# RoyiAvital/QuadraticProgramSolver

Hardware: AMD Instinct MI355X
Metric: ADMM iterations/sec (higher is better)
Workload: dtype f64

## Files before the change

quadraticprogramsolver_amd/csrc/k_loop.hip:

```cpp
#include <cstdlib>

#include "qps_kernels.h"
#include "wave_reduce.h"
#include <hip/hip_ext.h>

namespace qps {

namespace {

template <typename T> __device__ __forceinline__ T wave_sum(T v) { return wave_sum_all(v); }
__device__ __forceinline__ unsigned long long absbits(double v) { return (unsigned long long)__double_as_longlong(fabs(v)); }
__device__ __forceinline__ unsigned long long wave_max_u64(unsigned long long v) {
#pragma unroll
    for (int o = 32; o > 0; o >>= 1) { unsigned long long t = __shfl_xor(v, o, 64); v = t > v ? t : v; }
    return v;
}

template <typename T, int RB, int TRI, int THREADS>
__global__ __launch_bounds__(THREADS) void k_gemv_rows(const T* __restrict__ S, int64_t ld, const T* __restrict__ v,
                                                   T* __restrict__ out, const T* __restrict__ out0, T alpha, T beta,
                                                   int r0, int c0, int c1, BatchStride bs) {
    using V = typename VecOf<T>::type;
    if (bs.active && !bs.active[blockIdx.y]) return;
    S += (int64_t)blockIdx.y * bs.mat; v += (int64_t)blockIdx.y * bs.vin; out += (int64_t)blockIdx.y * bs.vout;
    if (out0) out0 += (int64_t)blockIdx.y * bs.vout;
    constexpr int VN = VecOf<T>::N;
// ... 9 lines not shown
    const T* Srow = S + (int64_t)rb * ld;
#pragma unroll 4
    for (int c = cb + tid * VN; c < ce; c += CHUNK) {
        const V vv = *reinterpret_cast<const V*>(v + c);
        const T* vp = reinterpret_cast<const T*>(&vv);
#pragma unroll
        for (int i = 0; i < RB; ++i) {
            typedef T NV __attribute__((ext_vector_type(VN)));
            const NV* src = reinterpret_cast<const NV*>(Srow + (int64_t)i * ld + c);
            const NV a = (TRI == 0) ? __builtin_nontemporal_load(src) : *src;
            T ap[VN];
#pragma unroll
            for (int e = 0; e < VN; ++e) ap[e] = a[e];
#pragma unroll
            for (int e = 0; e < VN; ++e) {
                bool ok = true;
                if (TRI == 1) ok = (c + e) <= (rb + i);
                if (TRI == 2) ok = (c + e) >= (rb + i);
                acc[i] += ok ? ap[e] * vp[e] : T(0);
            }
        }
    }
    __shared__ T red[THREADS / 64][RB];
#pragma unroll
    for (int i = 0; i < RB; ++i) acc[i] = wave_sum(acc[i]);
    if ((tid & 63) == 0) {
#pragma unroll
        for (int i = 0; i < RB; ++i) red[tid >> 6][i] = acc[i];
    }
    __syncthreads();
// ... 27 lines not shown
        T w = ca * va[rbase + i];
        if (vb) w += cb * vb[rbase + i];
        typedef T NV __attribute__((ext_vector_type(VN)));
        const NV a = __builtin_nontemporal_load(reinterpret_cast<const NV*>(Sp + (int64_t)i * ld));
#pragma unroll
        for (int e = 0; e < VN; ++e) acc[e] += a[e] * w;
    }
    V o;
    T* op = reinterpret_cast<T*>(&o);
#pragma unroll
    for (int e = 0; e < VN; ++e) op[e] = acc[e];
    *reinterpret_cast<V*>(part + (int64_t)rt * part_ld + c) = o;
}

template <typename T>
__global__ __launch_bounds__(256) void k_colsum(const T* __restrict__ part, int64_t part_ld, int ntiles,
                                                const T* __restrict__ a0, T s0, const T* __restrict__ a1, T s1,
                                                T* __restrict__ out, int ncols, BatchStride bs) {
    using V = typename VecOf<T>::type;
    constexpr int VN = VecOf<T>::N;
    if (bs.active && !bs.active[blockIdx.y]) return;
    part += (int64_t)blockIdx.y * bs.mat; out += (int64_t)blockIdx.y * bs.vout;
    if (a0) a0 += (int64_t)blockIdx.y * bs.vin;
    if (a1) a1 += (int64_t)blockIdx.y * bs.vin;
    constexpr int COLS = 128 / (int)sizeof(T);
    constexpr int CL = COLS / VN;
    constexpr int TL = 256 / CL;
    const int cl = threadIdx.x % CL, tl = threadIdx.x / CL;
    const int c = blockIdx.x * COLS + cl * VN;
    T acc[VN];
#pragma unroll
    for (int e = 0; e < VN; ++e) acc[e] = T(0);
    if (c < ncols) {
        int t = tl;
        for (; t + 7 * TL < ntiles; t += 8 * TL) {
            V v[8];
#pragma unroll
            for (int j = 0; j < 8; ++j) v[j] = *reinterpret_cast<const V*>(part + (int64_t)(t + TL * j) * part_ld + c);
#pragma unroll
// ... 10 lines not shown
            for (int e = 0; e < VN; ++e) acc[e] += vp[e];
        }
    }
    __shared__ T red[TL][COLS + 1];
#pragma unroll
    for (int e = 0; e < VN; ++e) red[tl][cl * VN + e] = acc[e];
    __syncthreads();
    constexpr int PL = 256 / COLS;
    static_assert(TL % PL == 0 && (PL == 16 || PL == 8), "slab lanes per output");
    const int o = threadIdx.x / PL, pl = threadIdx.x % PL;
    T s = T(0);
#pragma unroll
    for (int k = 0; k < TL / PL; ++k) s += red[pl * (TL / PL) + k][o];
    s = (PL == 16) ? row16_sum_last(s) : oct_sum_all(s);
    const int oc = blockIdx.x * COLS + o;
    if (pl == PL - 1 && oc < ncols) {
        T r = s;
        if (a0) r += s0 * a0[oc];
        if (a1) r += s1 * a1[oc];
        out[oc] = r;
    }
}

template <typename T>
__global__ __launch_bounds__(256) void k_admm_update(int NP, int MP, const T* __restrict__ xx, const T* __restrict__ zz,
                                                     T* __restrict__ x, T* __restrict__ xp, T* __restrict__ z,
                                                     T* __restrict__ zp, T* __restrict__ y, const T* __restrict__ l,
                                                     const T* __restrict__ u, T alpha, T rho) {
    const int i = blockIdx.x * 256 + threadIdx.x;
    const T alpha1 = T(1) - alpha, rho1 = T(1) / rho;
    if (i < NP) {
        const T xo = x[i];
        xp[i] = xo;
        x[i] = alpha * xx[i] + alpha1 * xo;
    }
    if (i < MP) {
// ... 34 lines not shown
            v[4] = max(v[4], absbits((double)Px[i]));
            v[5] = max(v[5], absbits((double)Aty[i]));
            v[6] = max(v[6], absbits((double)q[i]));
            if (!dual_only) v[7] = max(v[7], absbits((double)(x[i] - xp[i])));
        }
    }
#pragma unroll
    for (int k = 0; k < 9; ++k) {
        v[k] = wave_max_u64(v[k]);
        if ((threadIdx.x & 63) == 0 && v[k] != 0ull) atomicMax(&slots[k], v[k]);
    }
}

__device__ __forceinline__ double jmax(double a, double b) { return (isnan(a) || isnan(b)) ? (double)NAN : (a > b ? a : b); }

__global__ void k_check_decide(const unsigned long long* __restrict__ slots, double* __restrict__ res, CheckScalars cs,
                               const double* __restrict__ rho_arr, const double* __restrict__ rhorho_arr,
                               const int* __restrict__ active) {
    if (threadIdx.x != 0) return;
    const int b = blockIdx.x;
    if (active && !active[b]) return;
    slots += (int64_t)b * 16; res += (int64_t)b * 8;
    if (rho_arr) { cs.rho = rho_arr[b]; cs.rhorho = rhorho_arr[b]; cs.convFlag = 1; }
    double nv[9];
    for (int k = 0; k < 9; ++k) nv[k] = __longlong_as_double((long long)slots[k]);
    const double MIN_VAL_RHO = 1e-3, MAX_VAL_RHO = 1e6;
    const double normResPrim = nv[0], normResDual = nv[1];
    const double maxNormPrim = jmax(nv[2], nv[3]);
    const double maxNormDual = jmax(jmax(nv[4], nv[5]), nv[6]);
    double rhorho = cs.rhorho;
    if (cs.adptRho) {
        const double numeratorVal = normResPrim * maxNormDual;
        const double denominatorVal = normResDual * maxNormPrim;
        const double t = cs.rho * sqrt(numeratorVal / denominatorVal);
        rhorho = t > MAX_VAL_RHO ? MAX_VAL_RHO : (t < MIN_VAL_RHO ? MIN_VAL_RHO : t);
    }
    const double epsPrim = cs.epsAbs + cs.epsRel * maxNormPrim;
    const double epsDual = cs.epsAbs + cs.epsRel * maxNormDual;
    int flag = cs.convFlag;
    if ((normResPrim < epsPrim) && (normResDual < epsDual)) flag = 3;
    if ((nv[7] <= cs.epsAdmm) && (nv[8] <= cs.epsAdmm)) flag = 2;
    res[0] = normResPrim; res[1] = normResDual; res[2] = maxNormPrim; res[3] = maxNormDual;
    res[4] = rhorho; res[5] = (double)flag; res[6] = nv[7]; res[7] = nv[8];
}

template <typename T> __global__ void k_fill(T* p, int64_t n, T v) {
    int64_t i = (int64_t)blockIdx.x * 256 + threadIdx.x;
    if (i < n) p[i] = v;
}
template <typename T> __global__ void k_convert(const double* __restrict__ s, T* __restrict__ d, int64_t n) {
    int64_t i = (int64_t)blockIdx.x * 256 + threadIdx.x;
    if (i < n) d[i] = (T)s[i];
}
template <typename T> __global__ void k_convert_back(const T* __restrict__ s, double* __restrict__ d, int64_t n) {
    int64_t i = (int64_t)blockIdx.x * 256 + threadIdx.x;
    if (i < n) d[i] = (double)s[i];
}

// ... 59 lines not shown
}

template <typename T>
void check_convergence(hipStream_t st, int n, int m, const T* Ax, const T* Px, const T* Aty, const T* q, const T* x,
                       const T* xp, const T* z, const T* zp, unsigned long long* scratch, double* res_dev, CheckScalars cs,
                       int dual_only, BatchStride bs, const double* rho_arr, const double* rhorho_arr) {
    if (!dual_only) (void)hipMemsetAsync(scratch, 0, 16 * sizeof(unsigned long long) * bs.count, st);
    const int N = n > m ? n : m;
    int blocks = (N + 255) / 256;
    if (blocks > 1024) blocks = 1024;
    if (blocks < 1) blocks = 1;
    hipLaunchKernelGGL((k_check_norms<T>), dim3(blocks, bs.count), dim3(256), 0, st, n, m, Ax, Px, Aty, q, x, xp, z, zp, scratch, dual_only, bs);
    hipLaunchKernelGGL(k_check_decide, dim3(bs.count), dim3(64), 0, st, scratch, res_dev, cs, rho_arr, rhorho_arr, bs.active);
}

template <typename T> void fill(hipStream_t st, T* p, int64_t n, T v) {
    if (n <= 0) return;
    hipLaunchKernelGGL((k_fill<T>), dim3((unsigned)((n + 255) / 256)), dim3(256), 0, st, p, n, v);
}
template <typename T> void convert_copy(hipStream_t st, const double* src, T* dst, int64_t n) {
    if (n <= 0) return;
    hipLaunchKernelGGL((k_convert<T>), dim3((unsigned)((n + 255) / 256)), dim3(256), 0, st, src, dst, n);
}
template <typename T> void convert_back(hipStream_t st, const T* src, double* dst, int64_t n) {
    if (n <= 0) return;
    hipLaunchKernelGGL((k_convert_back<T>), dim3((unsigned)((n + 255) / 256)), dim3(256), 0, st, src, dst, n);
}

#define INST(T)                                                                                                              \
    template void gemv_rows<T>(hipStream_t, const T*, int64_t, const T*, T*, const T*, T, T, int, int, int, int, int, BatchStride); \
    template int gemv_cols_partial<T>(hipStream_t, const T*, int64_t, const T*, const T*, T, T, T*, int64_t, int, int);      \
    template void colsum<T>(hipStream_t, const T*, int64_t, int, const T*, T, const T*, T, T*, int, BatchStride);            \
    template void admm_update<T>(hipStream_t, int, int, const T*, const T*, T*, T*, T*, T*, T*, const T*, const T*, T, T);   \
    template void check_convergence<T>(hipStream_t, int, int, const T*, const T*, const T*, const T*, const T*, const T*,    \
                                       const T*, const T*, unsigned long long*, double*, CheckScalars, int, BatchStride,     \
                                       const double*, const double*);                                                        \
    template void fill<T>(hipStream_t, T*, int64_t, T);                                                                      \
    template void convert_copy<T>(hipStream_t, const double*, T*, int64_t);                                                  \
    template void convert_back<T>(hipStream_t, const T*, double*, int64_t);
INST(double)
INST(float)
#undef INST

}
```

quadraticprogramsolver_amd/csrc/qps_capi.hip:

```cpp
#include "ldl_symbolic.h"
#include <atomic>
#include <limits>
#include <memory>
#include <thread>

#include "batch_schedule.h"
#include "dense_chol.h"
#include "qps_internal.h"
#include "spmv_layout.h"
#include "qps_kernels.h"
#include "qps_ldl.h"
#include "qps_polish.h"
#include "qps_proxqp.h"

using namespace qps;

namespace qps {
namespace {
constexpr size_t kPinnedBytes = 512, kRecycleBlockMax = (size_t)512 << 20;
constexpr int kRecyclePerDevice = 4;
std::mutex g_res_mu;
std::vector<HandleResources> g_res[kMaxDevices];
std::atomic<int> g_cus[kMaxDevices];
}
// ... 95 lines not shown
template <typename T> struct DenseSolver : SolverBase {
    int NP = 0, MP = 0;
    T *A = nullptr, *P = nullptr, *q = nullptr, *l = nullptr, *u = nullptr;
    T *PI = nullptr, *AA = nullptr, *M = nullptr, *S = nullptr, *tmp = nullptr, *dinv = nullptr; int* fail = nullptr;
    T *x = nullptr, *xp = nullptr, *z = nullptr, *zp = nullptr, *y = nullptr, *xx = nullptr, *zz = nullptr, *tt = nullptr, *yv = nullptr;
    T *part = nullptr, *part2 = nullptr, *sw_part = nullptr, *Ax = nullptr, *Px = nullptr, *Aty = nullptr;
    T* At = nullptr; void* small_out = nullptr; void* small_out_host = nullptr; bool small_ok = false;
    StreamLease lease; Arena arena;
    double* stage_mat = nullptr; int64_t stage_mat_count = 0;
    int pass_slabs = 0, pass_rpw = 0;
    unsigned long long* scratch = nullptr; double* res_dev = nullptr; double* res_host = nullptr; double* stage = nullptr;
    bool have_AA = false, factor_valid = false; double fac_rho = 0, fac_sigma = 0; int fac_nb = 0;
    int nb = 2048; int part_tiles = 0; int num_factorizations = 0;
    unsigned long long* pub = nullptr; unsigned* abort_dev = nullptr; unsigned sweep_epoch = 0; bool blocked_off = false, fac_premul = false;
    bool use_blocked() const { return !blocked_off && trsv_blocked_supported<T>(NP, nb); }
    struct IterGraph { int count; const void* xa; double rho, sigma, alpha; int nb; hipGraphExec_t exec; };
    std::vector<IterGraph> graphs;
    bool graphs_disabled = false;
    void drop_graphs() { for (auto& gr : graphs) (void)hipGraphExecDestroy(gr.exec); graphs.clear(); }
    hipGraphExec_t iter_graph(int count, T* xa, T* xb, double rho, double sigma, double alpha) {
        for (auto& gr : graphs) if (gr.count == count && gr.xa == xa && gr.rho == rho && gr.sigma == sigma && gr.alpha == alpha && gr.nb == nb) return gr.exec;
        if (graphs_disabled) return nullptr;
        if (graphs.size() >= 8) drop_graphs();
        hipGraph_t graph = nullptr; hipGraphExec_t exec = nullptr;
        if (hipStreamBeginCapture(st, hipStreamCaptureModeThreadLocal) != hipSuccess) { (void)hipGetLastError(); graphs_disabled = true; return nullptr; }
        for (int k = 0; k < count; ++k) {
            colsum<T>(st, part, NP, pass_slabs, xa, (T)sigma, q, T(-1), tt, NP);
            sweeps();
            apass<T>(st, false, A, NP, NP, MP, xx, xa, xb, z, y, l, u, (T)alpha, (T)rho, part, part2, NP, scratch);
            std::swap(xa, xb);
// ... 32 lines not shown
            Ax = ar.take<T>(MP); Px = ar.take<T>(NP); Aty = ar.take<T>(NP);
            scratch = ar.take<unsigned long long>(16); res_dev = ar.take<double>(16);
            pub = ar.take<unsigned long long>(trsv_blocked_pub_words<T>(NP));
            abort_dev = reinterpret_cast<unsigned*>(res_dev + 14);
            stage = ar.take<double>((int64_t)NP + 2 * (int64_t)MP + 64);
            if (small_ok) { At = ar.take<T>((int64_t)NP * MP); small_out = ar.take<double>(32); }
            if (stage_mat_count > 0) stage_mat = ar.take<double>(stage_mat_count);
        };
        layout(arena);
        st = prof.st = lease.acquire(device, arena.planned());
        HandleResources& res = lease.res;
        char* const recycled = res.block; res.block = nullptr;
        arena.commit(st, recycled, res.block_bytes);
        layout(arena);
        res_host = reinterpret_cast<double*>(res.pinned);
        small_out_host = small_ok ? reinterpret_cast<char*>(res.pinned) + 16 * sizeof(double) : nullptr;
        const double s = sizeof(T);
        cat_atw = prof.category("gemv_cols(A'w)", s * ((double)m * n + m + n));
        cat_colsum = prof.category("colsum(rhs)", s * ((double)part_tiles * n + 3.0 * n));
        cat_fwd = prof.category("trsv_forward", s * ((double)n * (n + 1) / 2 + 2.0 * n));
        cat_bwd = prof.category("trsv_backward", s * ((double)n * (n + 1) / 2 + 2.0 * n));
        cat_ax = prof.category("gemv_rows(Ax~)", s * ((double)m * n + m + n));
        cat_upd = prof.category("admm_update", s * (3.0 * n + 7.0 * m));
        cat_chk = prof.category("check_convergence", s * (2.0 * m * n + (double)n * n + 4.0 * n + 4.0 * m));
        cat_pass = prof.category("apass(fused A-pass)", s * ((double)m * n + 3.0 * n + 6.0 * m));
        cat_passchk = prof.category("apass(check variant)", s * ((double)m * n + 4.0 * n + 6.0 * m));
        cat_sweep = prof.category("sweeps(fused fwd+bwd, triangle read once)", s * ((double)n * (n + 1) / 2 + 2.0 * n + (double)sweep_fused_slabs<T>(NP) * n));
        cat_xsum = prof.category("colsum(x~ slabs)", s * ((double)sweep_fused_slabs<T>(NP) * n + n));
        cat_small = prof.category("admm_small(whole loop in one launch; bytes per iteration)", s * ((double)m * n + (double)n * n) + s * (6.0 * n + 10.0 * m));
    }
// ... 132 lines not shown
            ii = it;
            const double t2s = now_s();
            PolishReport prs;
            if (p.polish) polish_dense<T>(st, n, m, NP, MP, P, A, q, l, u, y, x, part, p, &prs);
            download_vec(x, xh, n);
            if (info) {
                info->convFlag = convFlag; info->iterations = ii; info->numRefactor = nref; info->cgIterations = 0;
                info->rhoFinal = rho; info->rhoProposed = rhorho; info->resPrim = resP; info->resDual = resD;
                info->tSetup = t1 - t0; info->tLoop = t2s - t1; info->tRefactor = tref;
                info->polishFlag = prs.flag; info->polishIterations = prs.minresIterations; info->tPolish = prs.seconds;
                info->trsvBlock = nb; info->sweepVariant = 4;
            }
            return false;
        }
        const bool fused = pass_slabs > 0 && p.loopVariant != 1;
        int rhs_slabs = 0;
        static const int graph_env = [] { const char* e = getenv("QPS_GRAPH"); return e ? atoi(e) : -1; }();
        const bool use_graph = fused && prof.level == 0 && p.numItrConv >= 3 && !fac_premul && (graph_env >= 0 ? graph_env != 0 : NP <= 2048);
        for (ii = 1; ii <= p.numIterations; ++ii) {
            bool changed = false;
            if (p.adptRho && ((rhorho * p.fctrRho < rho) || (rhorho > p.fctrRho * rho))) {
                rho = rhorho; ++nref; changed = true;
                const double ta = now_s();
                factorize(rho, sigma, false);
                tref += now_s() - ta;
            }
            const bool check = (ii % p.numItrConv == 0);
            if (use_graph && !changed && !check && rhs_slabs == pass_slabs) {
                int run = std::min(p.numItrConv - ii % p.numItrConv, p.numIterations - ii + 1) & ~1;
                hipGraphExec_t ge = run >= 2 ? iter_graph(run, x, xp, rho, sigma, alpha) : nullptr;
// ... 5 lines not shown
            }
            if (!fused) {
                linear_solve(rho, sigma);
                {
                    ProfScope ps(prof, cat_upd, 2);
                    admm_update<T>(st, NP, MP, xx, zz, x, xp, z, zp, y, l, u, (T)alpha, (T)rho);
                }
                if (check) {
                    ProfScope ps(prof, cat_chk, 2);
                    gemv_rows<T>(st, A, NP, x, Ax, nullptr, T(1), T(0), 0, MP, 0, NP, 0);
                    gemv_rows<T>(st, P, NP, x, Px, nullptr, T(1), T(0), 0, NP, 0, NP, 0);
                    gemv_cols_partial<T>(st, A, NP, y, nullptr, T(1), T(0), part, NP, MP, NP);
                    colsum<T>(st, part, NP, part_tiles, nullptr, T(0), nullptr, T(0), Aty, NP);
                    CheckScalars cs{p.epsAbs, p.epsRel, epsAdmm, rho, rhorho, p.adptRho, convFlag};
                    check_convergence<T>(st, (int)n, (int)m, Ax, Px, Aty, q, x, xp, z, zp, scratch, res_dev, cs);
                }
            } else {
                if (changed && rhs_slabs > 0) {
                    ProfScope ps(prof, cat_atw, 2);
                    rhs_slabs = gemv_cols_partial<T>(st, A, NP, z, y, (T)rho, T(-1), part, NP, MP, NP);
                }
                prof_iter = ii;
                {
                    ProfLaunchScope ps(prof, cat_colsum, sample_lvl(29));
                    colsum<T>(st, part, NP, rhs_slabs, x, (T)sigma, q, T(-1), tt, NP);
                }
                sweeps();
                if (check) HIPC(hipMemsetAsync(scratch, 0, 16 * sizeof(unsigned long long), st));
                {
                    const int lvl = (prof.level == 1 && (check || ii % 50 != 38)) ? 3 : 1;
                    ProfLaunchScope ps(prof, check ? cat_passchk : cat_pass, lvl);
                    apass<T>(st, check, A, NP, NP, MP, xx, x, xp, z, y, l, u, (T)alpha, (T)rho, part, part2, NP, scratch);
                }
                std::swap(x, xp);
                rhs_slabs = pass_slabs;
                if (check) {
                    ProfScope ps(prof, cat_chk, 2);
                    colsum<T>(st, part2, NP, pass_slabs, nullptr, T(0), nullptr, T(0), Aty, NP);
                    gemv_rows<T>(st, P, NP, x, Px, nullptr, T(1), T(0), 0, NP, 0, NP, 0);
                    CheckScalars cs{p.epsAbs, p.epsRel, epsAdmm, rho, rhorho, p.adptRho, convFlag};
                    check_convergence<T>(st, (int)n, (int)m, Ax, Px, Aty, q, x, xp, z, zp, scratch, res_dev, cs, 1);
                }
            }
            if (check) {
                HIPC(hipMemcpyAsync(res_host, res_dev, 15 * sizeof(double), hipMemcpyDeviceToHost, st));
                HIPC(hipStreamSynchronize(st));
                prof.harvest();
                if (sweep_gave_up(true)) return true;
                resP = res_host[0]; resD = res_host[1]; rhorho = res_host[4]; convFlag = (int)res_host[5];
                if (convFlag != QPS_CONV_NUM_ITR) break;
            }
        }
        HIPC(hipStreamSynchronize(st));
        prof.harvest();
        if (sweep_gave_up()) return true;
        const double t2 = now_s();
        PolishReport pr;
        if (p.polish) polish_dense<T>(st, n, m, NP, MP, P, A, q, l, u, y, x, part, p, &pr);
        download_vec(x, xh, n);
        if (info) {
            info->convFlag = convFlag; info->iterations = ii > p.numIterations ? p.numIterations : ii;
// ... 104 lines not shown
    const double denominatorVal = res[8 * bd + 1] * res[8 * bp + 2];
    const double t = rho * std::sqrt(numeratorVal / denominatorVal);
    return t > MAX_VAL_RHO ? MAX_VAL_RHO : (t < MIN_VAL_RHO ? MIN_VAL_RHO : t);
}

template <typename T> struct BatchedDenseSolver : BatchSolverBase {
    StreamLease lease; DeviceOwner mem; hipStream_t st = nullptr;
    int NP = 0, MP = 0, nb = 0, slabs = 0, rpw = 0, part_tiles = 0;
    T *A = nullptr, *P = nullptr, *q = nullptr, *l = nullptr, *u = nullptr, *PI = nullptr, *AA = nullptr, *M = nullptr, *S = nullptr,
      *tmp = nullptr, *dinv = nullptr;
    T *x = nullptr, *xp = nullptr, *xres = nullptr, *z = nullptr, *y = nullptr, *xx = nullptr, *tt = nullptr, *yv = nullptr, *part = nullptr,
      *part2 = nullptr, *part_tmp = nullptr, *sw_part = nullptr, *Px = nullptr, *Aty = nullptr;
    int* fail = nullptr; int* d_active = nullptr; double *d_rho = nullptr, *d_rhorho = nullptr;
    unsigned long long* scratch = nullptr; double* res_dev = nullptr; double* res_host = nullptr; double* stage = nullptr;
    int* h_int = nullptr; double* h_dbl = nullptr;
    bool have_AA = false; double fac_sigma = -1; int fac_nb = -1; std::vector<double> fac_rho;
    char* sb_args = nullptr; void* sb_host = nullptr;
    int cat_pass = 0, cat_sweep = 0;

    BatchedDenseSolver(int dev, int cnt, int64_t n_, int64_t m_) {
        device = dev; n = n_; m = m_; count = cnt;
        HIPC(hipSetDevice(device));
        st = prof.st = lease.acquire(device);
        NP = roundup(n, 64); MP = roundup(m, 64);
        slabs = apass_plan<T>(NP, MP, &rpw, count);
        {
            const double s = sizeof(T), c = cnt;
            cat_pass = prof.category("apass(fused A-pass, batched)", c * s * ((double)m * n + 3.0 * n + 6.0 * m));
            cat_sweep = prof.category("sweeps(fused fwd+bwd, batched, triangle read once)", c * s * ((double)n * (n + 1) / 2 + 2.0 * n));
        }
        part_tiles = gemv_cols_tiles(MP);
        const int64_t nn = (int64_t)NP * NP, c = count;
        A = mem.dalloc<T>(c * MP * NP, st); P = mem.dalloc<T>(c * nn, st); PI = mem.dalloc<T>(c * nn, st); AA = mem.dalloc<T>(c * nn, st); M = mem.dalloc<T>(c * nn, st);
        S = mem.dalloc<T>(c * nn, st); tmp = mem.dalloc<T>(c * nn, st); dinv = mem.dalloc<T>(c * (int64_t)(NP / 64) * 4096, st);
        q = mem.dalloc<T>(c * NP, st); l = mem.dalloc<T>(c * MP, st); u = mem.dalloc<T>(c * MP, st);
        x = mem.dalloc<T>(c * NP, st); xp = mem.dalloc<T>(c * NP, st); xres = mem.dalloc<T>(c * NP, st); xx = mem.dalloc<T>(c * NP, st); tt = mem.dalloc<T>(c * NP, st);
        yv = mem.dalloc<T>(c * NP, st); Px = mem.dalloc<T>(c * NP, st); Aty = mem.dalloc<T>(c * NP, st); z = mem.dalloc<T>(c * MP, st); y = mem.dalloc<T>(c * MP, st);
        int rpw1 = 0;
        const int64_t part_slabs = std::max<int64_t>(std::max<int64_t>(c * slabs, apass_plan<T>(NP, MP, &rpw1, 1)), std::max(part_tiles, 1));
        part = mem.dalloc<T>(part_slabs * NP, st); part2 = mem.dalloc<T>(c * slabs * NP, st); part_tmp = mem.dalloc<T>((int64_t)std::max(part_tiles, 1) * NP, st);
        const int sw_slabs = sweep_fused_slabs<T>(NP, count); sw_part = mem.dalloc<T>(c * std::max(sw_slabs, 1) * NP, st);
        fail = mem.dalloc<int>(count + 4, st); d_active = mem.dalloc<int>(count + 4, st); d_rho = mem.dalloc<double>(count + 4, st); d_rhorho = mem.dalloc<double>(count + 4, st);
        scratch = mem.dalloc<unsigned long long>(16 * c, st); res_dev = mem.dalloc<double>(8 * c, st);
        res_host = mem.pinned<double>(8 * c); h_int = mem.pinned<int>(count + 4); h_dbl = mem.pinned<double>(2 * (count + 4));
        stage = mem.dalloc<double>(std::max<int64_t>((int64_t)MP * NP, nn) + 64, st);
    }
    ~BatchedDenseSolver() override {
        (void)hipSetDevice(device);
        (void)hipStreamSynchronize(st);
        prof.release_events();
    }
    std::unique_ptr<FastUploader> loader;
    void put_vec(const double* h, T* d, int64_t cnt_) {
        if (cnt_ <= 0) return;
        if (!loader) loader.reset(new FastUploader(st, device));
        loader->copy(stage, h, sizeof(double) * (size_t)cnt_);
        convert_copy<T>(st, stage, d, cnt_);
    }
    void put_matrix(const double* h, int rows, int cols, T* d) {
// ... 46 lines not shown
        else for (int b : todo) { ch.at(b).form(sigma, p.rho, rebuild, rebuild); ch.at(b).factor(nb); }
        ch.check(what, "", h_int, count, &todo);
        have_AA = true; fac_sigma = sigma; fac_nb = nb;
        for (int b : todo) fac_rho[b] = p.rho;
        for (int b = 0; b < count; ++b) put_vec(xh + (int64_t)b * n, x + (int64_t)b * NP, n);
        loader.reset();
        HIPC(hipMemsetAsync(z, 0, sizeof(T) * (size_t)count * MP, st));
        HIPC(hipMemsetAsync(y, 0, sizeof(T) * (size_t)count * MP, st));
        push_state(rho, rhorho, active);
        const double t1 = now_s();
        BatchStride bsS; bsS.count = count; bsS.mat = (int64_t)NP * NP; bsS.vin = NP; bsS.vout = NP; bsS.active = d_active;
        BatchStride bsC; bsC.count = count; bsC.mat = (int64_t)slabs * NP; bsC.vin = NP; bsC.vout = NP; bsC.active = d_active;
        BatchStride bsK; bsK.count = count; bsK.vin = NP; bsK.vout = MP; bsK.active = d_active;
        PassBatch pb; pb.count = count; pb.slabs = slabs; pb.rho_arr = d_rho; pb.active = d_active;
        int rhs_slabs = 0, nactive = count, ii = 0;
        const int nblk = (NP + nb - 1) / nb;
        if (p.loopVariant == 0 && nblk == 1 && admm_small_batch_supported<T>(NP, MP)) {
            const size_t ab = admm_small_args_bytes(), ob = admm_small_out_bytes();
            if (!sb_host) { sb_args = mem.dalloc<char>((int64_t)(ab + ob) * count + 64, st); sb_host = mem.pinned<char>((ab + ob) * (size_t)count + 64); }
            char* args_h = static_cast<char*>(sb_host); char* outs_h = args_h + ab * count;
            char* args_d = sb_args; char* outs_d = sb_args + ab * count;
            std::vector<int> it(count, 0);
            HIPC(hipMemsetAsync(xp, 0, sizeof(T) * (size_t)count * NP, st));
            while (nactive > 0) {
                for (int b = 0; b < count; ++b)
                    admm_small_args_set(args_h, b, (int)n, (int)m, NP, MP, it[b], active[b] ? p.numIterations : it[b], p.numItrConv, p.adptRho, rho[b], rhorho[b],
                                        sigma, alpha, p.epsAbs, p.epsRel, epsAdmm, p.fctrRho);
                HIPC(hipMemcpyAsync(args_d, args_h, ab * count, hipMemcpyHostToDevice, st));
                admm_small_batch<T>(st, count, NP, MP, args_d, A, P, S, q, l, u, x, xp, z, y, outs_d);
                HIPC(hipMemcpyAsync(outs_h, outs_d, ob * count, hipMemcpyDeviceToHost, st));
// ... 42 lines not shown
                    if (rhs_slabs > 0) {
                        T* pb_ = part + (int64_t)b * slabs * NP;
                        gemv_cols_partial<T>(st, A + (int64_t)b * MP * NP, NP, z + (int64_t)b * MP, y + (int64_t)b * MP, (T)rho[b], T(-1), part_tmp, NP, MP, NP);
                        colsum<T>(st, part_tmp, NP, part_tiles, nullptr, T(0), nullptr, T(0), pb_, NP);
                        if (slabs > 1) HIPC(hipMemsetAsync(pb_ + NP, 0, sizeof(T) * (size_t)(slabs - 1) * NP, st));
                    }
                }
                ch.check(what, "", h_int, count, together ? &all : &changed);
                push_state(rho, rhorho, active);
                const double dt = (now_s() - ta) / changed.size();
                for (int b : changed) tref[b] += dt;
            }
            const bool check = (ii % p.numItrConv == 0);
            colsum<T>(st, part, NP, rhs_slabs, x, (T)sigma, q, T(-1), tt, NP, bsC);
            ch.sweeps(nb, tt, yv, xx, sw_part, bsS, {&prof, cat_sweep, (prof.level == 1 && ii % 50 == 13) ? 1 : 2});
            if (check) HIPC(hipMemsetAsync(scratch, 0, 16 * sizeof(unsigned long long) * count, st));
            {
                ProfLaunchScope ps(prof, cat_pass, (prof.level == 1 && !check && ii % 50 == 38) ? 1 : (check ? 3 : 2));
                apass<T>(st, check, A, NP, NP, MP, xx, x, xp, z, y, l, u, (T)alpha, T(1), part, part2, NP, scratch, pb);
            }
            std::swap(x, xp);
            rhs_slabs = slabs;
            if (check) {
                colsum<T>(st, part2, NP, slabs, nullptr, T(0), nullptr, T(0), Aty, NP, bsC);
                BatchStride bsP = bsS; bsP.mat = (int64_t)NP * NP;
                gemv_rows<T>(st, P, NP, x, Px, nullptr, T(1), T(0), 0, NP, 0, NP, 0, bsP);
                CheckScalars cs{p.epsAbs, p.epsRel, epsAdmm, 0.0, 0.0, p.adptRho, QPS_CONV_NUM_ITR};
                check_convergence<T>(st, (int)n, (int)m, (const T*)nullptr, Px, Aty, q, x, xp, z, z, scratch, res_dev, cs, 1, bsK, d_rho, d_rhorho);
                HIPC(hipMemcpyAsync(res_host, res_dev, 8 * sizeof(double) * count, hipMemcpyDeviceToHost, st));
                HIPC(hipStreamSynchronize(st));
                prof.harvest();
                bool any_done = false;
                for (int b = 0; b < count; ++b) {
                    if (!active[b]) continue;
                    const double* r = res_host + 8 * b;
                    resP[b] = r[0]; resD[b] = r[1]; rhorho[b] = r[4]; conv[b] = (int)r[5];
                    if (conv[b] != QPS_CONV_NUM_ITR) {
                        active[b] = 0; iters[b] = ii; --nactive; any_done = true;
                        HIPC(hipMemcpyAsync(xres + (int64_t)b * NP, x + (int64_t)b * NP, sizeof(T) * NP, hipMemcpyDeviceToDevice, st));
                    }
                }
                push_state(rho, rhorho, active);
                (void)any_done;
            }
        }
// ... 1266 lines not shown
```

quadraticprogramsolver_amd/csrc/qps_internal.h:

```cpp
#pragma once
#include <hip/hip_runtime.h>

#include <algorithm>
#include <chrono>
#include <cmath>
#include <cstdio>
#include <cstring>
#include <mutex>
#include <string>
#include <system_error>
#include <thread>
#include <vector>

#include "../../include/qps.h"

namespace qps {

struct QpsError { int code; std::string msg; QpsError(int c, std::string m) : code(c), msg(std::move(m)) {} };

inline double now_s() { return std::chrono::duration<double>(std::chrono::steady_clock::now().time_since_epoch()).count(); }
inline int roundup(int64_t v, int q) { return (int)(((v + q - 1) / q) * q); }

struct KernelStat { double seconds = 0; int64_t launches = 0; double algo_bytes = 0; };

// ... 27 lines not shown
        for (auto& p : pending) { (void)hipEventDestroy(p.a); (void)hipEventDestroy(p.b); }
        pool.clear(); pending.clear();
    }
    ~Profiler() { for (auto e : pool) (void)hipEventDestroy(e); for (auto& p : pending) { (void)hipEventDestroy(p.a); (void)hipEventDestroy(p.b); } }
};
struct ProfLaunchScope {
    Profiler& p; int cat; hipEvent_t a, b; bool active;
    ProfLaunchScope(Profiler& pr, int c, int lvl);
    ~ProfLaunchScope();
};
struct ProfScope {
    Profiler& p; int cat; hipEvent_t a; bool active;
    ProfScope(Profiler& pr, int c, int lvl) : p(pr), cat(c), a(nullptr), active(pr.on(lvl)) { if (active) p.begin(cat, a); }
    ~ProfScope() { if (active) p.end(cat, a); }
};

#define HIPC(expr)                                                                                            \
    do {                                                                                                      \
        hipError_t e_ = (expr);                                                                               \
        if (e_ != hipSuccess) {                                                                               \
            char b_[512]; snprintf(b_, sizeof b_, "%s failed: %s (%s:%d)", #expr, hipGetErrorString(e_), __FILE__, __LINE__); \
            throw QpsError(e_ == hipErrorOutOfMemory ? QPS_ERR_OUT_OF_MEMORY : QPS_ERR_HIP, b_);               \
        }                                                                                                     \
    } while (0)

struct DeviceOwner {
    std::vector<void*> dev, host;
    DeviceOwner() = default;
    DeviceOwner(const DeviceOwner&) = delete;
    DeviceOwner& operator=(const DeviceOwner&) = delete;
// ... 151 lines not shown
```

quadraticprogramsolver_amd/csrc/qps_kernels.h:

```cpp
#pragma once
#ifndef QPS_NT_SLABS
#define QPS_NT_SLABS 1
#endif
#include <hip/hip_runtime.h>
#include <stdint.h>

#include <atomic>
#include <thread>

namespace qps {

constexpr int kMaxDevices = 64;
int current_device();
int device_cu_count(int device);
struct PerDeviceOnce {
    std::atomic<unsigned char> state[kMaxDevices] = {};
    template <typename F> void once(int dev, F&& f) {
        if (dev < 0 || dev >= kMaxDevices) { f(); return; }
        if (state[dev].load(std::memory_order_acquire) == 2) return;
        unsigned char expect = 0;
        if (state[dev].compare_exchange_strong(expect, 1, std::memory_order_acq_rel)) { f(); state[dev].store(2, std::memory_order_release); return; }
        while (state[dev].load(std::memory_order_acquire) != 2) std::this_thread::yield();
    }
};
// ... 19 lines not shown

template <typename T>
void colsum(hipStream_t st, const T* part, int64_t part_ld, int ntiles, const T* a0, T s0, const T* a1, T s1,
            T* out, int ncols, BatchStride bs = BatchStride());

template <typename T>
void admm_update(hipStream_t st, int NP, int MP, const T* xx, const T* zz, T* x, T* xp, T* z, T* zp, T* y,
                 const T* l, const T* u, T alpha, T rho);

struct CheckScalars { double epsAbs, epsRel, epsAdmm, rho, rhorho; int adptRho; int convFlag; };
template <typename T>
void check_convergence(hipStream_t st, int n, int m, const T* Ax, const T* Px, const T* Aty, const T* q, const T* x,
                       const T* xp, const T* z, const T* zp, unsigned long long* scratch , double* res_dev,
                       CheckScalars cs, int dual_only = 0, BatchStride bs = BatchStride(), const double* rho_arr = nullptr,
                       const double* rhorho_arr = nullptr);

template <typename T> int apass_plan(int NP, int MP, int* rows_per_wg, int count = 1);
template <typename T> int apass_max_np();
struct PassBatch { int count = 1; int slabs = 0; const double* rho_arr = nullptr; const int* active = nullptr; int pq_me = 0; };
template <typename T>
void apass(hipStream_t st, bool check, const T* A, int64_t ld, int NP, int MP, const T* xx, const T* x_old, T* x_new, T* z,
           T* y, const T* l, const T* u, T alpha, T rho, T* part, T* part2, int64_t part_ld, unsigned long long* slots,
           PassBatch pb = PassBatch());
template <typename T> int apass_proxqp_slabs(int NP, int MP);
template <typename T>
int apass_kkt(hipStream_t st, const T* A, int64_t ld, int NP, int MP, const T* vx, const T* vlam, const T* mask, T delta, T* out_lam,
              T* part, int64_t part_ld);
template <typename T>
int apass_proxqp(hipStream_t st, const T* G, int64_t ld, int NP, int MP, int me, const T* x, T* x_scratch, T* slack, T* dual,
                 const T* g, T rho, T* part, int64_t part_ld);
// ... 106 lines not shown
```

Measured before the change: 14510.

## Fuse convergence-check colsum, P*x gemv and decide into one epilogue kernel

Adds a k_check_epilogue kernel that, in one launch, reduces the A'y partial sums, computes P*x with double-buffered loads, folds in the dual-residual max norms, and has the last workgroup (chosen by an atomic ticket) run the convergence decision. It writes results straight into mapped pinned host memory and resets the slot scratch itself, so the memset and the device-to-host copy can be skipped on later checks. It also switches the untriangular gemv inner loop to explicit FMA. This removes several kernel launches and a memcpy per check iteration, at the cost of a more complex kernel that relies on cross-workgroup atomic ordering and on zero-copy host writes.

```diff
diff --git a/quadraticprogramsolver_amd/csrc/k_loop.hip b/quadraticprogramsolver_amd/csrc/k_loop.hip
--- a/quadraticprogramsolver_amd/csrc/k_loop.hip
+++ b/quadraticprogramsolver_amd/csrc/k_loop.hip
@@ -10,6 +10,8 @@
 
 template <typename T> __device__ __forceinline__ T wave_sum(T v) { return wave_sum_all(v); }
 __device__ __forceinline__ unsigned long long absbits(double v) { return (unsigned long long)__double_as_longlong(fabs(v)); }
+__device__ __forceinline__ double fmadd(double a, double b, double c) { return __builtin_fma(a, b, c); }
+__device__ __forceinline__ float fmadd(float a, float b, float c) { return __builtin_fmaf(a, b, c); }
 __device__ __forceinline__ unsigned long long wave_max_u64(unsigned long long v) {
 #pragma unroll
     for (int o = 32; o > 0; o >>= 1) { unsigned long long t = __shfl_xor(v, o, 64); v = t > v ? t : v; }
@@ -49,6 +51,7 @@
             for (int e = 0; e < VN; ++e) ap[e] = a[e];
 #pragma unroll
             for (int e = 0; e < VN; ++e) {
+                if (TRI == 0) { acc[i] = fmadd(ap[e], vp[e], acc[i]); continue; }
                 bool ok = true;
                 if (TRI == 1) ok = (c + e) <= (rb + i);
                 if (TRI == 2) ok = (c + e) >= (rb + i);
@@ -106,15 +109,10 @@
 }
 
 template <typename T>
-__global__ __launch_bounds__(256) void k_colsum(const T* __restrict__ part, int64_t part_ld, int ntiles,
-                                                const T* __restrict__ a0, T s0, const T* __restrict__ a1, T s1,
-                                                T* __restrict__ out, int ncols, BatchStride bs) {
+__device__ __forceinline__ T colsum_body(const T* __restrict__ part, int64_t part_ld, int ntiles, const T* __restrict__ a0, T s0,
+                                         const T* __restrict__ a1, T s1, T* __restrict__ out, int ncols, int* owner_col) {
     using V = typename VecOf<T>::type;
     constexpr int VN = VecOf<T>::N;
-    if (bs.active && !bs.active[blockIdx.y]) return;
-    part += (int64_t)blockIdx.y * bs.mat; out += (int64_t)blockIdx.y * bs.vout;
-    if (a0) a0 += (int64_t)blockIdx.y * bs.vin;
-    if (a1) a1 += (int64_t)blockIdx.y * bs.vin;
     constexpr int COLS = 128 / (int)sizeof(T);
     constexpr int CL = COLS / VN;
     constexpr int TL = 256 / CL;
@@ -155,12 +153,26 @@
     for (int k = 0; k < TL / PL; ++k) s += red[pl * (TL / PL) + k][o];
     s = (PL == 16) ? row16_sum_last(s) : oct_sum_all(s);
     const int oc = blockIdx.x * COLS + o;
+    *owner_col = -1;
+    T r = s;
     if (pl == PL - 1 && oc < ncols) {
-        T r = s;
         if (a0) r += s0 * a0[oc];
         if (a1) r += s1 * a1[oc];
         out[oc] = r;
-    }
+        *owner_col = o;
+    }
+    return r;
+}
+template <typename T>
+__global__ __launch_bounds__(256) void k_colsum(const T* __restrict__ part, int64_t part_ld, int ntiles,
+                                                const T* __restrict__ a0, T s0, const T* __restrict__ a1, T s1,
+                                                T* __restrict__ out, int ncols, BatchStride bs) {
+    if (bs.active && !bs.active[blockIdx.y]) return;
+    part += (int64_t)blockIdx.y * bs.mat; out += (int64_t)blockIdx.y * bs.vout;
+    if (a0) a0 += (int64_t)blockIdx.y * bs.vin;
+    if (a1) a1 += (int64_t)blockIdx.y * bs.vin;
+    int owner;
+    (void)colsum_body<T>(part, part_ld, ntiles, a0, s0, a1, s1, out, ncols, &owner);
 }
 
 template <typename T>
@@ -225,6 +237,26 @@
 
 __device__ __forceinline__ double jmax(double a, double b) { return (isnan(a) || isnan(b)) ? (double)NAN : (a > b ? a : b); }
 
+__device__ __forceinline__ void check_decide_body(const double* nv, const CheckScalars& cs, double* __restrict__ res) {
+    const double MIN_VAL_RHO = 1e-3, MAX_VAL_RHO = 1e6;
+    const double normResPrim = nv[0], normResDual = nv[1];
+    const double maxNormPrim = jmax(nv[2], nv[3]);
+    const double maxNormDual = jmax(jmax(nv[4], nv[5]), nv[6]);
+    double rhorho = cs.rhorho;
+    if (cs.adptRho) {
+        const double numeratorVal = normResPrim * maxNormDual;
+        const double denominatorVal = normResDual * maxNormPrim;
+        const double t = cs.rho * sqrt(numeratorVal / denominatorVal);
+        rhorho = t > MAX_VAL_RHO ? MAX_VAL_RHO : (t < MIN_VAL_RHO ? MIN_VAL_RHO : t);
+    }
+    const double epsPrim = cs.epsAbs + cs.epsRel * maxNormPrim;
+    const double epsDual = cs.epsAbs + cs.epsRel * maxNormDual;
+    int flag = cs.convFlag;
+    if ((normResPrim < epsPrim) && (normResDual < epsDual)) flag = 3;
+    if ((nv[7] <= cs.epsAdmm) && (nv[8] <= cs.epsAdmm)) flag = 2;
+    res[0] = normResPrim; res[1] = normResDual; res[2] = maxNormPrim; res[3] = maxNormDual;
+    res[4] = rhorho; res[5] = (double)flag; res[6] = nv[7]; res[7] = nv[8];
+}
 __global__ void k_check_decide(const unsigned long long* __restrict__ slots, double* __restrict__ res, CheckScalars cs,
                                const double* __restrict__ rho_arr, const double* __restrict__ rhorho_arr,
                                const int* __restrict__ active) {
@@ -235,24 +267,120 @@
     if (rho_arr) { cs.rho = rho_arr[b]; cs.rhorho = rhorho_arr[b]; cs.convFlag = 1; }
     double nv[9];
     for (int k = 0; k < 9; ++k) nv[k] = __longlong_as_double((long long)slots[k]);
-    const double MIN_VAL_RHO = 1e-3, MAX_VAL_RHO = 1e6;
-    const double normResPrim = nv[0], normResDual = nv[1];
-    const double maxNormPrim = jmax(nv[2], nv[3]);
-    const double maxNormDual = jmax(jmax(nv[4], nv[5]), nv[6]);
-    double rhorho = cs.rhorho;
-    if (cs.adptRho) {
-        const double numeratorVal = normResPrim * maxNormDual;
-        const double denominatorVal = normResDual * maxNormPrim;
-        const double t = cs.rho * sqrt(numeratorVal / denominatorVal);
-        rhorho = t > MAX_VAL_RHO ? MAX_VAL_RHO : (t < MIN_VAL_RHO ? MIN_VAL_RHO : t);
-    }
-    const double epsPrim = cs.epsAbs + cs.epsRel * maxNormPrim;
-    const double epsDual = cs.epsAbs + cs.epsRel * maxNormDual;
-    int flag = cs.convFlag;
-    if ((normResPrim < epsPrim) && (normResDual < epsDual)) flag = 3;
-    if ((nv[7] <= cs.epsAdmm) && (nv[8] <= cs.epsAdmm)) flag = 2;
-    res[0] = normResPrim; res[1] = normResDual; res[2] = maxNormPrim; res[3] = maxNormDual;
-    res[4] = rhorho; res[5] = (double)flag; res[6] = nv[7]; res[7] = nv[8];
+    check_decide_body(nv, cs, res);
+}
+
+constexpr int CE_RB = 4;
+constexpr int CE_UC = 4;
+template <typename T, bool WIDE>
+__global__ __launch_bounds__(256) void k_check_epilogue(const T* __restrict__ part2, int64_t part_ld, int ntiles, T* __restrict__ Aty,
+                                                        const T* __restrict__ P, int64_t ld, const T* __restrict__ x, T* __restrict__ Px,
+                                                        const T* __restrict__ q, int n, int NP, unsigned long long* __restrict__ slots,
+                                                        double* __restrict__ res, const unsigned* __restrict__ abort_src,
+                                                        unsigned* __restrict__ abort_dst, CheckScalars cs,
+                                                        const double* __restrict__ rho_arr, const double* __restrict__ rhorho_arr, BatchStride bs) {
+    constexpr int VN = VecOf<T>::N;
+    constexpr int COLS = 128 / (int)sizeof(T);
+    static_assert(COLS % CE_RB == 0 && COLS <= 64 && CE_UC % 2 == 0, "the norms of a workgroup's rows are reduced by its first wave");
+    const int b = blockIdx.y, tid = threadIdx.x;
+    if (bs.active && !bs.active[b]) return;
+    part2 += (int64_t)b * bs.mat; Aty += (int64_t)b * bs.vout; P += (int64_t)b * NP * ld;
+    x += (int64_t)b * bs.vin; Px += (int64_t)b * bs.vout; q += (int64_t)b * bs.vin; slots += (int64_t)b * 16; res += (int64_t)b * 8;
+    __shared__ T s_aty[COLS];
+    constexpr int NH = WIDE ? 2 : 1;
+    __shared__ T s_dot[COLS][4 * NH];
+    typedef T NV __attribute__((ext_vector_type(VN)));
+    constexpr int TRIP = CE_UC * 256 * VN;
+    const int rb0 = blockIdx.x * COLS;
+    const int ntrip = (NP + TRIP - 1) / TRIP, ntile = (COLS / CE_RB) * ntrip;
+    auto load_tile = [&](int j, NV (&a)[CE_RB][CE_UC], NV (&xv)[CE_UC]) {
+        const int g = j / ntrip, c0 = (j - g * ntrip) * TRIP + tid * VN;
+        const T* Prow = P + (int64_t)(rb0 + g * CE_RB) * ld;
+#pragma unroll
+        for (int k = 0; k < CE_UC; ++k) {
+            const int c = c0 + k * 256 * VN;
+            const bool in = c < NP;
+            xv[k] = in ? *reinterpret_cast<const NV*>(x + c) : NV(T(0));
+#pragma unroll
+            for (int i = 0; i < CE_RB; ++i)
+                a[i][k] = in ? __builtin_nontemporal_load(reinterpret_cast<const NV*>(Prow + (int64_t)i * ld + c)) : NV(T(0));
+        }
+    };
+    T acc[NH][CE_RB];
+#pragma unroll
+    for (int h = 0; h < NH; ++h)
+#pragma unroll
+        for (int i = 0; i < CE_RB; ++i) acc[h][i] = T(0);
+    auto use_tile = [&](int j, const NV (&a)[CE_RB][CE_UC], const NV (&xv)[CE_UC]) {
+#pragma unroll
+        for (int k = 0; k < CE_UC; ++k)
+#pragma unroll
+            for (int i = 0; i < CE_RB; ++i)
+#pragma unroll
+                for (int e = 0; e < VN; ++e) acc[k % NH][i] = fmadd(a[i][k][e], xv[k][e], acc[k % NH][i]);
+        const int g = j / ntrip;
+        if (j - g * ntrip != ntrip - 1) return;
+#pragma unroll
+        for (int h = 0; h < NH; ++h)
+#pragma unroll
+            for (int i = 0; i < CE_RB; ++i) {
+                const T w = wave_sum(acc[h][i]);
+                if ((tid & 63) == 0) s_dot[g * CE_RB + i][4 * h + (tid >> 6)] = w;
+                acc[h][i] = T(0);
+            }
+    };
+    NV a0[CE_RB][CE_UC], x0[CE_UC], a1[CE_RB][CE_UC], x1[CE_UC];
+    load_tile(0, a0, x0);
+    {
+        int owner;
+        const T r = colsum_body<T>(part2, part_ld, ntiles, (const T*)nullptr, T(0), (const T*)nullptr, T(0), Aty, NP, &owner);
+        if (owner >= 0) s_aty[owner] = r;
+    }
+    for (int j = 0; j < ntile; j += 2) {
+        if (j + 1 < ntile) load_tile(j + 1, a1, x1);
+        use_tile(j, a0, x0);
+        if (j + 1 < ntile) {
+            if (j + 2 < ntile) load_tile(j + 2, a0, x0);
+            use_tile(j + 1, a1, x1);
+        }
+    }
+    __syncthreads();
+    if (tid < 64) {
+        unsigned long long v1 = 0ull, v4 = 0ull, v5 = 0ull, v6 = 0ull;
+        if (tid < COLS) {
+            const int r = rb0 + tid;
+            T px = T(0);
+#pragma unroll
+            for (int w = 0; w < 4 * NH; ++w) px += s_dot[tid][w];
+            Px[r] = px;
+            if (r < n) {
+                const T aty = s_aty[tid], qq = q[r];
+                v1 = absbits((double)(px + qq + aty));
+                v4 = absbits((double)px); v5 = absbits((double)aty); v6 = absbits((double)qq);
+            }
+        }
+        v1 = wave_max_u64(v1); v4 = wave_max_u64(v4); v5 = wave_max_u64(v5); v6 = wave_max_u64(v6);
+        if (tid == 0) {
+            if (v1) atomicMax(&slots[1], v1);
+            if (v4) atomicMax(&slots[4], v4);
+            if (v5) atomicMax(&slots[5], v5);
+            if (v6) atomicMax(&slots[6], v6);
+            asm volatile("s_waitcnt vmcnt(0)" ::: "memory");
+            unsigned* ticket = reinterpret_cast<unsigned*>(slots + 15);
+            if (atomicAdd(ticket, 1u) == gridDim.x - 1u) {
+                double nv[9];
+#pragma unroll
+                for (int k = 0; k < 9; ++k)
+                    nv[k] = __longlong_as_double((long long)__hip_atomic_load(&slots[k], __ATOMIC_RELAXED, __HIP_MEMORY_SCOPE_AGENT));
+                if (rho_arr) { cs.rho = rho_arr[b]; cs.rhorho = rhorho_arr[b]; cs.convFlag = 1; }
+                check_decide_body(nv, cs, res);
+                if (abort_dst && abort_dst != abort_src)
+                    *abort_dst = __hip_atomic_load(abort_src, __ATOMIC_RELAXED, __HIP_MEMORY_SCOPE_AGENT);
+#pragma unroll
+                for (int k = 0; k < 16; ++k) __hip_atomic_store(&slots[k], 0ull, __ATOMIC_RELAXED, __HIP_MEMORY_SCOPE_AGENT);
+            }
+        }
+    }
 }
 
 template <typename T> __global__ void k_fill(T* p, int64_t n, T v) {
@@ -342,6 +470,21 @@
     hipLaunchKernelGGL(k_check_decide, dim3(bs.count), dim3(64), 0, st, scratch, res_dev, cs, rho_arr, rhorho_arr, bs.active);
 }
 
+template <typename T>
+void check_epilogue(hipStream_t st, int n, int NP, const T* part2, int64_t part_ld, int ntiles, const T* P, int64_t ld, const T* x, const T* q,
+                    T* Aty, T* Px, unsigned long long* scratch, double* res, const unsigned* abort_src, unsigned* abort_dst, CheckScalars cs,
+                    BatchStride bs, const double* rho_arr, const double* rhorho_arr) {
+    constexpr int cols_wg = 128 / (int)sizeof(T);
+    const dim3 grid((NP + cols_wg - 1) / cols_wg, bs.count);
+    if (NP >= 4 * 256 * VecOf<T>::N)
+        hipLaunchKernelGGL((k_check_epilogue<T, true>), grid, dim3(256), 0, st, part2, part_ld, ntiles, Aty, P, ld, x, Px, q, n, NP, scratch, res, abort_src, abort_dst,
+                           cs, rho_arr, rhorho_arr, bs);
+    else
+        hipLaunchKernelGGL((k_check_epilogue<T, false>), grid, dim3(256), 0, st, part2, part_ld, ntiles, Aty, P, ld, x, Px, q, n, NP, scratch, res, abort_src, abort_dst,
+                           cs, rho_arr, rhorho_arr, bs);
+}
+bool check_fused_enabled() { static const bool on = env_int("QPS_CHECK_FUSED", 1) != 0; return on; }
+
 template <typename T> void fill(hipStream_t st, T* p, int64_t n, T v) {
     if (n <= 0) return;
     hipLaunchKernelGGL((k_fill<T>), dim3((unsigned)((n + 255) / 256)), dim3(256), 0, st, p, n, v);
@@ -363,6 +506,9 @@
     template void check_convergence<T>(hipStream_t, int, int, const T*, const T*, const T*, const T*, const T*, const T*,    \
                                        const T*, const T*, unsigned long long*, double*, CheckScalars, int, BatchStride,     \
                                        const double*, const double*);                                                        \
+    template void check_epilogue<T>(hipStream_t, int, int, const T*, int64_t, int, const T*, int64_t, const T*, const T*, T*, T*,       \
+                                    unsigned long long*, double*, const unsigned*, unsigned*, CheckScalars, BatchStride,    \
+                                    const double*, const double*);                                                           \
     template void fill<T>(hipStream_t, T*, int64_t, T);                                                                      \
     template void convert_copy<T>(hipStream_t, const double*, T*, int64_t);                                                  \
     template void convert_back<T>(hipStream_t, const T*, double*, int64_t);
diff --git a/quadraticprogramsolver_amd/csrc/qps_capi.hip b/quadraticprogramsolver_amd/csrc/qps_capi.hip
--- a/quadraticprogramsolver_amd/csrc/qps_capi.hip
+++ b/quadraticprogramsolver_amd/csrc/qps_capi.hip
@@ -133,6 +133,7 @@
     int nb = 2048; int part_tiles = 0; int num_factorizations = 0;
     unsigned long long* pub = nullptr; unsigned* abort_dev = nullptr; unsigned sweep_epoch = 0; bool blocked_off = false, fac_premul = false;
     bool use_blocked() const { return !blocked_off && trsv_blocked_supported<T>(NP, nb); }
+    double* res_map = nullptr; bool slots_dirty = true;
     struct IterGraph { int count; const void* xa; double rho, sigma, alpha; int nb; hipGraphExec_t exec; };
     std::vector<IterGraph> graphs;
     bool graphs_disabled = false;
@@ -195,6 +196,7 @@
         arena.commit(st, recycled, res.block_bytes);
         layout(arena);
         res_host = reinterpret_cast<double*>(res.pinned);
+        res_map = map_pinned<double>(res_host);
         small_out_host = small_ok ? reinterpret_cast<char*>(res.pinned) + 16 * sizeof(double) : nullptr;
         const double s = sizeof(T);
         cat_atw = prof.category("gemv_cols(A'w)", s * ((double)m * n + m + n));
@@ -357,6 +359,9 @@
             return false;
         }
         const bool fused = pass_slabs > 0 && p.loopVariant != 1;
+        const bool chk_fused = fused && check_fused_enabled();
+        prof.stats[cat_chk].algo_bytes = chk_fused ? sizeof(T) * ((double)n * n + (double)pass_slabs * n + 6.0 * n)
+                                                   : sizeof(T) * (2.0 * m * n + (double)n * n + 4.0 * n + 4.0 * m);
         int rhs_slabs = 0;
         static const int graph_env = [] { const char* e = getenv("QPS_GRAPH"); return e ? atoi(e) : -1; }();
         const bool use_graph = fused && prof.level == 0 && p.numItrConv >= 3 && !fac_premul && (graph_env >= 0 ? graph_env != 0 : NP <= 2048);
@@ -392,6 +397,7 @@
                     colsum<T>(st, part, NP, part_tiles, nullptr, T(0), nullptr, T(0), Aty, NP);
                     CheckScalars cs{p.epsAbs, p.epsRel, epsAdmm, rho, rhorho, p.adptRho, convFlag};
                     check_convergence<T>(st, (int)n, (int)m, Ax, Px, Aty, q, x, xp, z, zp, scratch, res_dev, cs);
+                    slots_dirty = true;
                 }
             } else {
                 if (changed && rhs_slabs > 0) {
@@ -404,7 +410,8 @@
                     colsum<T>(st, part, NP, rhs_slabs, x, (T)sigma, q, T(-1), tt, NP);
                 }
                 sweeps();
-                if (check) HIPC(hipMemsetAsync(scratch, 0, 16 * sizeof(unsigned long long), st));
+                if (check && (!chk_fused || slots_dirty)) HIPC(hipMemsetAsync(scratch, 0, 16 * sizeof(unsigned long long), st));
+                if (check) slots_dirty = true;
                 {
                     const int lvl = (prof.level == 1 && (check || ii % 50 != 38)) ? 3 : 1;
                     ProfLaunchScope ps(prof, check ? cat_passchk : cat_pass, lvl);
@@ -414,15 +421,21 @@
                 rhs_slabs = pass_slabs;
                 if (check) {
                     ProfScope ps(prof, cat_chk, 2);
-                    colsum<T>(st, part2, NP, pass_slabs, nullptr, T(0), nullptr, T(0), Aty, NP);
-                    gemv_rows<T>(st, P, NP, x, Px, nullptr, T(1), T(0), 0, NP, 0, NP, 0);
                     CheckScalars cs{p.epsAbs, p.epsRel, epsAdmm, rho, rhorho, p.adptRho, convFlag};
-                    check_convergence<T>(st, (int)n, (int)m, Ax, Px, Aty, q, x, xp, z, zp, scratch, res_dev, cs, 1);
+                    if (chk_fused) {
+                        check_epilogue<T>(st, (int)n, NP, part2, NP, pass_slabs, P, NP, x, q, Aty, Px, scratch, res_map ? res_map : res_dev, abort_dev,
+                                          res_map ? reinterpret_cast<unsigned*>(res_map + 14) : abort_dev, cs);
+                    } else {
+                        colsum<T>(st, part2, NP, pass_slabs, nullptr, T(0), nullptr, T(0), Aty, NP);
+                        gemv_rows<T>(st, P, NP, x, Px, nullptr, T(1), T(0), 0, NP, 0, NP, 0);
+                        check_convergence<T>(st, (int)n, (int)m, Ax, Px, Aty, q, x, xp, z, zp, scratch, res_dev, cs, 1);
+                    }
                 }
             }
             if (check) {
-                HIPC(hipMemcpyAsync(res_host, res_dev, 15 * sizeof(double), hipMemcpyDeviceToHost, st));
+                if (!(chk_fused && res_map)) HIPC(hipMemcpyAsync(res_host, res_dev, 15 * sizeof(double), hipMemcpyDeviceToHost, st));
                 HIPC(hipStreamSynchronize(st));
+                if (chk_fused) slots_dirty = false;
                 prof.harvest();
                 if (sweep_gave_up(true)) return true;
                 resP = res_host[0]; resD = res_host[1]; rhorho = res_host[4]; convFlag = (int)res_host[5];
@@ -557,6 +570,7 @@
     int* fail = nullptr; int* d_active = nullptr; double *d_rho = nullptr, *d_rhorho = nullptr;
     unsigned long long* scratch = nullptr; double* res_dev = nullptr; double* res_host = nullptr; double* stage = nullptr;
     int* h_int = nullptr; double* h_dbl = nullptr;
+    double* res_map = nullptr; bool slots_dirty = true;
     bool have_AA = false; double fac_sigma = -1; int fac_nb = -1; std::vector<double> fac_rho;
     char* sb_args = nullptr; void* sb_host = nullptr;
     int cat_pass = 0, cat_sweep = 0;
@@ -586,6 +600,7 @@
         fail = mem.dalloc<int>(count + 4, st); d_active = mem.dalloc<int>(count + 4, st); d_rho = mem.dalloc<double>(count + 4, st); d_rhorho = mem.dalloc<double>(count + 4, st);
         scratch = mem.dalloc<unsigned long long>(16 * c, st); res_dev = mem.dalloc<double>(8 * c, st);
         res_host = mem.pinned<double>(8 * c); h_int = mem.pinned<int>(count + 4); h_dbl = mem.pinned<double>(2 * (count + 4));
+        res_map = map_pinned<double>(res_host);
         stage = mem.dalloc<double>(std::max<int64_t>((int64_t)MP * NP, nn) + 64, st);
     }
     ~BatchedDenseSolver() override {
@@ -662,6 +677,7 @@
         BatchStride bsK; bsK.count = count; bsK.vin = NP; bsK.vout = MP; bsK.active = d_active;
         PassBatch pb; pb.count = count; pb.slabs = slabs; pb.rho_arr = d_rho; pb.active = d_active;
         int rhs_slabs = 0, nactive = count, ii = 0;
+        const bool chk_fused = check_fused_enabled();
         const int nblk = (NP + nb - 1) / nb;
         if (p.loopVariant == 0 && nblk == 1 && admm_small_batch_supported<T>(NP, MP)) {
             const size_t ab = admm_small_args_bytes(), ob = admm_small_out_bytes();
@@ -734,7 +750,8 @@
             const bool check = (ii % p.numItrConv == 0);
             colsum<T>(st, part, NP, rhs_slabs, x, (T)sigma, q, T(-1), tt, NP, bsC);
             ch.sweeps(nb, tt, yv, xx, sw_part, bsS, {&prof, cat_sweep, (prof.level == 1 && ii % 50 == 13) ? 1 : 2});
-            if (check) HIPC(hipMemsetAsync(scratch, 0, 16 * sizeof(unsigned long long) * count, st));
+            if (check && (!chk_fused || slots_dirty)) HIPC(hipMemsetAsync(scratch, 0, 16 * sizeof(unsigned long long) * count, st));
+            if (check) slots_dirty = true;
             {
                 ProfLaunchScope ps(prof, cat_pass, (prof.level == 1 && !check && ii % 50 == 38) ? 1 : (check ? 3 : 2));
                 apass<T>(st, check, A, NP, NP, MP, xx, x, xp, z, y, l, u, (T)alpha, T(1), part, part2, NP, scratch, pb);
@@ -742,13 +759,18 @@
             std::swap(x, xp);
             rhs_slabs = slabs;
             if (check) {
-                colsum<T>(st, part2, NP, slabs, nullptr, T(0), nullptr, T(0), Aty, NP, bsC);
-                BatchStride bsP = bsS; bsP.mat = (int64_t)NP * NP;
-                gemv_rows<T>(st, P, NP, x, Px, nullptr, T(1), T(0), 0, NP, 0, NP, 0, bsP);
                 CheckScalars cs{p.epsAbs, p.epsRel, epsAdmm, 0.0, 0.0, p.adptRho, QPS_CONV_NUM_ITR};
-                check_convergence<T>(st, (int)n, (int)m, (const T*)nullptr, Px, Aty, q, x, xp, z, z, scratch, res_dev, cs, 1, bsK, d_rho, d_rhorho);
-                HIPC(hipMemcpyAsync(res_host, res_dev, 8 * sizeof(double) * count, hipMemcpyDeviceToHost, st));
+                if (chk_fused) {
+                    check_epilogue<T>(st, (int)n, NP, part2, NP, slabs, P, NP, x, q, Aty, Px, scratch, res_map ? res_map : res_dev, nullptr, nullptr, cs, bsC, d_rho, d_rhorho);
+                } else {
+                    colsum<T>(st, part2, NP, slabs, nullptr, T(0), nullptr, T(0), Aty, NP, bsC);
+                    BatchStride bsP = bsS; bsP.mat = (int64_t)NP * NP;
+                    gemv_rows<T>(st, P, NP, x, Px, nullptr, T(1), T(0), 0, NP, 0, NP, 0, bsP);
+                    check_convergence<T>(st, (int)n, (int)m, (const T*)nullptr, Px, Aty, q, x, xp, z, z, scratch, res_dev, cs, 1, bsK, d_rho, d_rhorho);
+                }
+                if (!(chk_fused && res_map)) HIPC(hipMemcpyAsync(res_host, res_dev, 8 * sizeof(double) * count, hipMemcpyDeviceToHost, st));
                 HIPC(hipStreamSynchronize(st));
+                if (chk_fused) slots_dirty = false;
                 prof.harvest();
                 bool any_done = false;
                 for (int b = 0; b < count; ++b) {
diff --git a/quadraticprogramsolver_amd/csrc/qps_internal.h b/quadraticprogramsolver_amd/csrc/qps_internal.h
--- a/quadraticprogramsolver_amd/csrc/qps_internal.h
+++ b/quadraticprogramsolver_amd/csrc/qps_internal.h
@@ -65,6 +65,13 @@
     ProfScope(Profiler& pr, int c, int lvl) : p(pr), cat(c), a(nullptr), active(pr.on(lvl)) { if (active) p.begin(cat, a); }
     ~ProfScope() { if (active) p.end(cat, a); }
 };
+
+template <typename T> inline T* map_pinned(T* host) {
+    void* d = nullptr;
+    if (host && hipHostGetDevicePointer(&d, host, 0) == hipSuccess) return static_cast<T*>(d);
+    (void)hipGetLastError();
+    return nullptr;
+}
 
 #define HIPC(expr)                                                                                            \
     do {                                                                                                      \
diff --git a/quadraticprogramsolver_amd/csrc/qps_kernels.h b/quadraticprogramsolver_amd/csrc/qps_kernels.h
--- a/quadraticprogramsolver_amd/csrc/qps_kernels.h
+++ b/quadraticprogramsolver_amd/csrc/qps_kernels.h
@@ -57,6 +57,12 @@
                        const T* xp, const T* z, const T* zp, unsigned long long* scratch , double* res_dev,
                        CheckScalars cs, int dual_only = 0, BatchStride bs = BatchStride(), const double* rho_arr = nullptr,
                        const double* rhorho_arr = nullptr);
+
+template <typename T>
+void check_epilogue(hipStream_t st, int n, int NP, const T* part2, int64_t part_ld, int ntiles, const T* P, int64_t ld, const T* x, const T* q,
+                    T* Aty, T* Px, unsigned long long* scratch, double* res, const unsigned* abort_src, unsigned* abort_dst, CheckScalars cs,
+                    BatchStride bs = BatchStride(), const double* rho_arr = nullptr, const double* rhorho_arr = nullptr);
+bool check_fused_enabled();
 
 template <typename T> int apass_plan(int NP, int MP, int* rows_per_wg, int count = 1);
 template <typename T> int apass_max_np();
```

New measurement: 14560 (median of 5 runs). No clear change (+0.4%).
